# KAIST-AILab/SyncVSR

Measured on AMD Instinct MI355X. Metric: lip-clips/sec training (29x88x88), higher is better.
Workload: dtype bf16; 1 GPU; LRW training step (fwd+bwd+allreduce+clip+AdamW), ResNet18 + 6-layer 512-d encoder + vq audio-token CE head, random-init weights, N(0,1) clips 29x88x88, uniform tokens/labels; per_gpu_batch=32, global_batch=32, parallelism=dp1, hip_graph=False, enqueue=native step list

## Files before the change

### include/syncvsr_hip.h

```cpp
#ifndef SYNCVSR_HIP_H
#define SYNCVSR_HIP_H

#include <stdint.h>

#ifndef __HIP_PLATFORM_AMD__
typedef void* hipStream_t;
#else
#include <hip/hip_runtime_api.h>
#endif

#define SVSR_OK 0
#define SVSR_ERR_ARG 1001
#define SVSR_GRAD_ADD_DW 1
#define SVSR_GRAD_ADD_DB 2
#define SVSR_ERR_GROUP_OPEN 1003
#define SVSR_ERR_NO_GROUP 1004
#define SVSR_ERR_MASK_SIZE 1005

typedef struct svsr_wgrad_problem {
    const void* x; const void* dy; float* dw; float* dbias; const int* plan_dev; const int* meta;
    int Nimg; int in_pix; int Ci; int in_pitch; int Co; int out_pix; int out_pitch; int wt_taps;
} svsr_wgrad_problem;

typedef struct svsr_enc_layer {
// ... 40 lines not shown
int svsr_conv3x3_c64_stat_rows(int Nimg, int H, int W);
int64_t svsr_conv3x3_c64_pixtab(int Nimg, int H, int W, int* out, int64_t cap);
int svsr_conv3x3_c64(const void* in, const void* wt, void* out, const void* addend, float* stats, int Nimg, int H, int W, const int* dy, const int* dx, const int* tw, const int* pixtab, hipStream_t stream);

int svsr_igemm_dgrad_bn(const void* in, const void* wt, void* out, const void* addend, float* stats, const int* plan_dev, const int* meta, int Nimg, int in_pix, int Ci, int in_pitch, int Co, int out_pix, int out_pitch, int wt_taps, const void* y, const void* x, const float* mean, const float* rstd, const float* gamma, const float* beta, int act, hipStream_t stream);
int svsr_igemm_dgrad_relu(const void* in, const void* wt, void* out, float* stats, const int* plan_dev, const int* meta, int Nimg, int in_pix, int Ci, int in_pitch, int Co, int out_pix, int out_pitch, int wt_taps, const void* y, const float* zeros, const float* ones, float gscale, hipStream_t stream);
int svsr_conv3x3_c64_dgrad_bn(const void* in, const void* wt, void* out, const void* addend, float* stats, int Nimg, int H, int W, const int* dy, const int* dx, const int* tw, const void* y, const void* x, const float* mean, const float* rstd, const float* gamma, const float* beta, int act, const int* pixtab, hipStream_t stream);
int svsr_bn_bwd_from_stats(const void* g, const void* x, const float* mean, const float* rstd, const float* gamma, const float* stats, int nrows, float* coef, float* dgamma, float* dbeta, void* dx, int64_t npix, int C, hipStream_t stream);


int svsr_conv3x3_wgrad_plan(int Nimg, int H, int W, int Ci, int Co, int* splits, int64_t* part_floats);
int svsr_conv3x3_wgrad(const void* x, const void* dy, float* dw, int Nimg, int H, int W, int Ci, int Co, float* part, int64_t part_floats, hipStream_t stream);
int svsr_conv3x3_wgrad_v2(const void* x, const void* dy, float* dw, int Nimg, int H, int W, int Ci, int Co, float* part, int64_t part_floats, int mode, hipStream_t stream);

int svsr_stem_conv_fwd_stat_rows(int B, int T, int H, int W);
int64_t svsr_stem_conv_fwd_ws_bytes(int B, int T, int H, int W);
int svsr_stem_conv_fwd(const float* vid, const float* w, void* out, float* stats, int B, int T, int H, int W, void* ws, int64_t ws_bytes, hipStream_t stream);

int svsr_stem_conv_wgrad_plan(int B, int T, int H, int W, int* splits, int64_t* part_floats);
int svsr_stem_conv_wgrad(const float* vid, const void* dy, float* dw, int B, int T, int H, int W, int use_tr, float* part, int64_t part_floats, hipStream_t stream);

int svsr_stem_bwd_wgrad_ok(int B, int T, int H, int W);
int svsr_stem_bwd_wgrad(const float* vid, const void* gpool, const void* amax, const void* x, const float* mean, const float* rstd, const float* coef, float* dw, int B, int T, int H, int W, float* part, int64_t part_floats, hipStream_t stream);

int svsr_bn_finalize(const float* part, int nrows, int C, float count, float eps, float momentum, float* mean, float* rstd, float* running_mean, float* running_var, int64_t* num_batches_tracked, hipStream_t stream);

int svsr_bn_eval_prepare(const float* running_mean, const float* running_var, int C, float eps, float* mean, float* rstd, hipStream_t stream);

int svsr_bn_act_fwd(const void* x, const void* res, void* y, const float* mean, const float* rstd, const float* gamma, const float* beta, int64_t npix, int C, int act, hipStream_t stream);

int svsr_bn_act_bwd_rows(int64_t npix, int C);
int svsr_bn_act_bwd(const void* dy, const void* y, const void* x, const float* mean, const float* rstd, const float* gamma, float* slots, float* coef, float* dgamma, float* dbeta, void* dx, void* dres, int64_t npix, int C, int act, const float* beta, const void* res, hipStream_t stream);

int svsr_stem_bn_act_pool_fwd(const void* x, void* y, void* amax, const float* mean, const float* rstd, const float* gamma, const float* beta, int N, int Hc, int Wc, int Hp, int Wp, int C, int act, void* xwin, hipStream_t stream);

int svsr_stem_bn_act_pool_bwd_rows(int N, int Hc, int Wc, int C);
int svsr_stem_bn_act_pool_bwd(const void* dpool, const void* amax, const void* x, const float* mean, const float* rstd, const float* gamma, const float* beta, float* slots, float* coef, float* dgamma, float* dbeta, void* dx, int N, int Hc, int Wc, int Hp, int Wp, int C, int act, const void* xwin, void* gpool, hipStream_t stream);

int svsr_avgpool_fwd(const void* x, void* y, int64_t N, int HW, int C, hipStream_t stream);
int svsr_avgpool_bwd(const void* dy, void* dx, int64_t N, int HW, int C, hipStream_t stream);

int svsr_add_ln_fwd(const void* a, const void* r, const float* gamma, const float* beta, void* y, float* mean, float* rstd, int R, int D, float eps, hipStream_t stream);
int svsr_add_ln_bwd_rows(int R);
int svsr_add_ln_bwd(const void* dy, const void* a, const void* r, const float* gamma, const float* mean, const float* rstd, void* ds, float* dgamma, float* dbeta, int R, int D, const void* addend, float* part, hipStream_t stream);
int svsr_add_ln_bwd_partials(const void* dy, const void* a, const void* r, const float* gamma, const float* mean, const float* rstd, void* ds, int R, int D, const void* addend, float* part, hipStream_t stream);
int svsr_add_ln_bwd_branch(const void* dy, const void* a, const void* r, const float* gamma, const float* mean, const float* rstd, void* ds, int R, int D, const void* addend, float* part, void* ds2, float alpha2, const unsigned* drop_seed, unsigned drop_site, float drop_p, hipStream_t stream);
// ... 165 lines not shown
```

### syncvsr_amd/build.py

```python
from __future__ import annotations

import glob
import os
import subprocess
import sys
from concurrent.futures import ThreadPoolExecutor

PKG = os.path.dirname(os.path.abspath(__file__))
CSRC = os.path.join(PKG, "csrc")
LIB = os.path.join(PKG, "libsyncvsr_hip.so")
OBJ = os.path.join(PKG, "csrc", "_obj")
ARCH = "gfx950"
FLAGS = ["-O3", "-std=c++17", "-fPIC", f"--offload-arch={ARCH}", "-Wno-unused-value", "-ffp-contract=fast"]


def _hipcc() -> str:
    for c in ("hipcc", "/opt/rocm/bin/hipcc"):
        try:
            subprocess.run([c, "--version"], capture_output=True, check=True)
            return c
        except (OSError, subprocess.CalledProcessError):
            continue
    raise RuntimeError("hipcc not found (needed to build the gfx950 kernels)")


def sources() -> list[str]:
    return sorted(glob.glob(os.path.join(CSRC, "*.hip")))


def headers() -> list[str]:
    pub = os.path.join(os.path.dirname(os.path.dirname(os.path.abspath(__file__))), "include")
    return glob.glob(os.path.join(CSRC, "*.h")) + glob.glob(os.path.join(pub, "*.h"))


VARIANTS = {"": [], "syncdbg": ["-DSVSR_SYNC_DEBUG"], "p8stamp": ["-DSVSR_P8_STAMP"]}


def lib_path(variant: str = "") -> str:
    return os.path.join(PKG, f"libsyncvsr_hip_{variant}.so") if variant else LIB


def stale(variant: str = "") -> bool:
    lib = lib_path(variant)
    if not os.path.exists(lib):
        return True
    t = os.path.getmtime(lib)
    deps = sources() + headers()
    return any(os.path.getmtime(d) > t for d in deps)


def build(force: bool = False, verbose: bool = True, variant: str = "") -> str:
    LIB = lib_path(variant)
    OBJ = os.path.join(PKG, "csrc", "_obj" + ("_" + variant if variant else ""))
    if not force and not stale(variant):
        return LIB
    cc = _hipcc()
    os.makedirs(OBJ, exist_ok=True)
    srcs = sources()
# ... 28 lines not shown
```

### syncvsr_amd/csrc/stem.hip

```cpp
#include "common.h"

#define STEM_C 64
#define STEM_KROWS 36
#define STEM_WPITCH 296

typedef __attribute__((ext_vector_type(4))) unsigned v4u;
typedef __attribute__((ext_vector_type(2))) unsigned v2u;

struct StemFwdArgs {
    const float* vid;
    const float* w;
    bf16_t* out;
    float* stats;
    int B, T, H, W, Ho, Wo;
    int tiles_per_frame, total_tiles;
    int rows_in_max, WP;
};

__global__ __launch_bounds__(256) void k_stem_conv_fwd(const StemFwdArgs p) {
    extern __shared__ __attribute__((aligned(16))) unsigned char smem_raw[];
    bf16_t* sW = reinterpret_cast<bf16_t*>(smem_raw);
    bf16_t* sIn = sW + STEM_C * STEM_WPITCH;
    const int tid = threadIdx.x, lane = tid & 63, wave = tid >> 6;
    const int HoWo = p.Ho * p.Wo;
// ... 517 lines not shown
            }
        }
        if (nxt >= p.total_tiles) break;
    }
    float* dst = p.part + (long)blockIdx.x * (STEM_C * 245);
#pragma unroll
    for (int q = 0; q < 2; ++q) {
        const int k = (wave * 2 + q) * 32 + (lane & 31);
        if (k >= 245) continue;
#pragma unroll
        for (int i = 0; i < 2; ++i)
#pragma unroll
            for (int r = 0; r < 16; ++r) {
                const int c = i * 32 + (r & 3) + 8 * (r >> 2) + 4 * (lane >> 5);
                dst[c * 245 + k] = acc[i][q][r];
            }
    }
}


#define SBW_PR (SW_RB / 2 + 1)
#define SBW_NG 3

struct StemBwdWgradArgs {
    const float* vid;
    const bf16_t* x;
    const bf16_t* gpool;
    const unsigned char* amax;
    const float* mean;
    const float* rstd;
    const float* coef;
    float* part;
    int B, T, H, W, Ho, Wo, Hp, Wp;
    int WoP, PW, groups_per_frame, total_tiles;
};

template <int NDY, int NIN>
__global__ __launch_bounds__(256, 2) void k_stem_bwd_wgrad(const StemBwdWgradArgs p) {
    extern __shared__ __attribute__((aligned(16))) unsigned char smem_raw[];
    constexpr int nrows = 2 * SW_RB + 5;
    bf16_t* sDY = reinterpret_cast<bf16_t*>(smem_raw);
    bf16_t* sIn = sDY + SW_RB * p.WoP * SW_DPITCH;
    bf16_t* sG = sIn + 5 * nrows * 2 * p.PW;
    unsigned char* sM = reinterpret_cast<unsigned char*>(sG + SBW_PR * p.Wp * STEM_C);
    float* sC = reinterpret_cast<float*>(sM + SBW_PR * p.Wp * STEM_C);
    const int tid_k = threadIdx.x, lane = tid_k & 63, wave = tid_k >> 6;
    const int kg = lane >> 5;

    int kbase[2];
    bool kvalid[2];
#pragma unroll
    for (int q = 0; q < 2; ++q) {
        const int k = (wave * 2 + q) * 32 + (lane & 31);
        kvalid[q] = k < 245;
        const int kk = kvalid[q] ? k : 0;
        const int kt = kk / 49, kh = (kk % 49) / 7, kw = kk % 7;
        const int plane = (kw + 1) & 1, off = (kw + 1) >> 1;
        kbase[q] = ((kt * nrows + kh) * 2 + plane) * p.PW + off + kg * 8;
    }

    f32x16 acc[2][2];
#pragma unroll
    for (int i = 0; i < 2; ++i)
#pragma unroll
        for (int j = 0; j < 2; ++j)
#pragma unroll
            for (int r = 0; r < 16; ++r) acc[i][j][r] = 0.f;

    v4u xv[NDY], gv[SBW_NG];
    v2u mv[SBW_NG];
    f32x4 inv[NIN];
    const int dy_total = SW_RB * p.WoP * 8, g_total = SBW_PR * p.Wp * 8;
    const int nq = p.W >> 2, in_total = 5 * nrows * nq;
    const float inv_nq = 1.f / (float)nq;
    for (int d = tid_k; d < 5 * nrows * p.PW; d += 256) reinterpret_cast<unsigned*>(sIn)[d] = 0u;
    if (tid_k < STEM_C) {
        sC[0 * STEM_C + tid_k] = p.mean[tid_k]; sC[1 * STEM_C + tid_k] = p.rstd[tid_k];
        sC[2 * STEM_C + tid_k] = p.coef[tid_k]; sC[3 * STEM_C + tid_k] = p.coef[STEM_C + tid_k]; sC[4 * STEM_C + tid_k] = p.coef[2 * STEM_C + tid_k];
    }
    const float inv_wop = 1.f / (float)p.WoP;

    for (int tile = (int)blockIdx.x - (int)gridDim.x;; tile += gridDim.x) {
        const int nxt = tile + (int)gridDim.x;
        int rb = 0;
        int tid = tid_k;
        asm volatile("" : "+v"(tid));
        const int c0 = (tid & 7) * 8;
        if (tile >= 0) {
            const int gi = tile % p.groups_per_frame, y0 = gi * SW_RB, p_lo = y0 >> 1;
            rb = p.Ho - y0;
            if (rb > SW_RB) rb = SW_RB;
            __syncthreads();
#pragma unroll
            for (int i = 0; i < NDY; ++i) {
                const int e = tid + 256 * i;
                if (e < dy_total) *reinterpret_cast<v4u*>(sDY + (e >> 3) * SW_DPITCH + c0) = xv[i];
            }
#pragma unroll
            for (int i = 0; i < SBW_NG; ++i) {
                const int e = tid + 256 * i;
                if (e < g_total) {
                    *reinterpret_cast<v4u*>(sG + (e >> 3) * STEM_C + c0) = gv[i];
                    *reinterpret_cast<v2u*>(sM + (e >> 3) * STEM_C + c0) = mv[i];
                }
            }
#pragma unroll
            for (int i = 0; i < NIN; ++i) {
                const int it = tid + 256 * i, rr = (int)(((float)it + 0.5f) * inv_nq), l = it - rr * nq;
                if (it < in_total) {
                    bf16_t* dst = sIn + (long)rr * 2 * p.PW;
                    reinterpret_cast<unsigned*>(dst)[l + 1] = pack2bf(inv[i][0], inv[i][2]);
                    reinterpret_cast<unsigned*>(dst + p.PW)[l + 1] = pack2bf(inv[i][1], inv[i][3]);
                }
            }
            __syncthreads();
            float mu[8], rs[8], k0[8], k1[8], k2[8];
#pragma unroll
            for (int k = 0; k < 8; ++k) {
                mu[k] = sC[0 * STEM_C + c0 + k]; rs[k] = sC[1 * STEM_C + c0 + k];
                k0[k] = sC[2 * STEM_C + c0 + k]; k1[k] = sC[3 * STEM_C + c0 + k]; k2[k] = sC[4 * STEM_C + c0 + k];
            }
            const int nbw = (p.Wo + 1) >> 1;
#pragma unroll 1
            for (int e = tid; e < (SW_RB / 2) * nbw * 8; e += 256) {
                const int blk = e >> 3, rp = blk >= nbw ? 1 : 0, cp = blk - rp * nbw;
                if (2 * rp >= rb) continue;
                const bool row1 = 2 * rp + 1 < rb, col1 = 2 * cp + 1 < p.Wo;
                const bool ph1 = p_lo + rp + 1 < p.Hp, pw1 = cp + 1 < p.Wp;
                const int soA = (rp * p.Wp + cp) * STEM_C + c0, soB = soA + (pw1 ? STEM_C : 0);
                const int soC = soA + (ph1 ? p.Wp * STEM_C : 0), soD = soC + (pw1 ? STEM_C : 0);
                const uint2 mA = *reinterpret_cast<const uint2*>(sM + soA), mB = *reinterpret_cast<const uint2*>(sM + soB);
                const uint2 mC = *reinterpret_cast<const uint2*>(sM + soC), mD = *reinterpret_cast<const uint2*>(sM + soD);
                float gA[8], gB[8], gC[8], gD[8];
                unpack8(*reinterpret_cast<const u32x4*>(sG + soA), gA);
                unpack8(*reinterpret_cast<const u32x4*>(sG + soB), gB);
                unpack8(*reinterpret_cast<const u32x4*>(sG + soC), gC);
                unpack8(*reinterpret_cast<const u32x4*>(sG + soD), gD);
                const unsigned offB = pw1 ? 0u : 0xffu, offC = ph1 ? 0u : 0xffu, offD = (ph1 && pw1) ? 0u : 0xffu;
// ... 6 lines not shown
    {                                                                                                              \
        bf16_t* cell = sDY + ((2 * rp + dy_) * p.WoP + 2 * cp + dx_) * SW_DPITCH + c0;                            \
        float xf[8], a[8], ov[8];                                                                                  \
        unpack8(*reinterpret_cast<const u32x4*>(cell), xf);                                                        \
        _Pragma("unroll") for (int k = 0; k < 8; ++k) a[k] = 0.f;                                               \
        BODY                                                                                                       \
        _Pragma("unroll") for (int k = 0; k < 8; ++k) {                                                         \
            const float xh = (xf[k] - mu[k]) * rs[k];                                                              \
            ov[k] = k0[k] * (a[k] - k1[k] - xh * k2[k]);                                                           \
        }                                                                                                          \
        *reinterpret_cast<u32x4*>(cell) = pack8(ov);                                                               \
        __builtin_amdgcn_sched_barrier(0);                                                                         \
    }
                SBW_ELEM(0, 0, SBW_WIN(a, mA, gA, 4u))
                if (col1) SBW_ELEM(0, 1, SBW_WIN(a, mA, gA, 5u) SBW_WIN(a, mB, gB, 3u | offB))
                if (row1) {
                    SBW_ELEM(1, 0, SBW_WIN(a, mA, gA, 7u) SBW_WIN(a, mC, gC, 1u | offC))
                    if (col1) SBW_ELEM(1, 1, SBW_WIN(a, mA, gA, 8u) SBW_WIN(a, mB, gB, 6u | offB) SBW_WIN(a, mC, gC, 2u | offC) SBW_WIN(a, mD, gD, 0u | offD))
                }
#undef SBW_ELEM
#undef SBW_WIN
            }
            __syncthreads();
        }
        {
        if (nxt < p.total_tiles) {
            const int f = nxt / p.groups_per_frame, gi = nxt - f * p.groups_per_frame;
            const int b = f / p.T, t = f - b * p.T;
            const int y0 = gi * SW_RB, p_lo = y0 >> 1;
            int rbn = p.Ho - y0;
            if (rbn > SW_RB) rbn = SW_RB;
            const int row_base = 2 * y0 - 3;
#pragma unroll
            for (int i = 0; i < NDY; ++i) {
                const int e = tid + 256 * i, pos = e >> 3, yl = (int)(((float)pos + 0.5f) * inv_wop), w = pos - yl * p.WoP;
                const bool ok = e < dy_total && yl < rbn && w < p.Wo;
                xv[i] = *reinterpret_cast<const v4u*>(ok ? p.x + (((long)f * p.Ho + y0 + yl) * p.Wo + w) * STEM_C + c0
                                                           : reinterpret_cast<const bf16_t*>(g_stem_zero));
            }
            const int g_live = (p.Hp - p_lo) * p.Wp * 8;
#pragma unroll
            for (int i = 0; i < SBW_NG; ++i) {
                const int e = tid + 256 * i;
                const bool ok = e < g_total && e < g_live;
                const long o = (((long)f * p.Hp + p_lo) * p.Wp + (e >> 3)) * STEM_C + c0;
                gv[i] = *reinterpret_cast<const v4u*>(ok ? p.gpool + o : reinterpret_cast<const bf16_t*>(g_stem_zero));
                mv[i] = *reinterpret_cast<const v2u*>(ok ? p.amax + o : reinterpret_cast<const unsigned char*>(g_stem_zero));
            }
#pragma unroll
            for (int i = 0; i < NIN; ++i) {
                const int it = tid + 256 * i, rr = (int)(((float)it + 0.5f) * inv_nq), l = it - rr * nq;
                const int kt = rr / nrows, r = rr - kt * nrows;
                const int tt = t + kt - 2, iy = row_base + r;
                const bool ok = it < in_total && tt >= 0 && tt < p.T && iy >= 0 && iy < p.H;
                inv[i] = *reinterpret_cast<const f32x4*>(ok ? p.vid + (((long)b * p.T + tt) * p.H + iy) * p.W + 4 * l
                                                             : reinterpret_cast<const float*>(g_stem_zero));
            }
        }
        }
        if (tile < 0) {
            if (nxt >= p.total_tiles) break;
            continue;
        }

        for (int yl = 0; yl < rb; ++yl) {
            for (int xs = 0; xs < p.WoP; xs += 16) {
                const int pos0 = yl * p.WoP + xs;
                bf16x8 fa[2], fb[2];
                fa[0] = stem_frag_T<true>(sDY, 0, pos0, lane);
                fa[1] = stem_frag_T<true>(sDY, 32, pos0, lane);
#pragma unroll
                for (int q = 0; q < 2; ++q) {
                    const int a = kbase[q] + (2 * yl) * 2 * p.PW + xs;
                    const unsigned* src = reinterpret_cast<const unsigned*>(sIn + (a & ~1));
                    const unsigned sh = (a & 1) * 16;
                    const unsigned d0 = src[0], d1 = src[1], d2 = src[2], d3 = src[3], d4 = src[4];
                    u32x4 fr;
                    fr.x = kvalid[q] ? __builtin_amdgcn_alignbit(d1, d0, sh) : 0u;
                    fr.y = kvalid[q] ? __builtin_amdgcn_alignbit(d2, d1, sh) : 0u;
                    fr.z = kvalid[q] ? __builtin_amdgcn_alignbit(d3, d2, sh) : 0u;
                    fr.w = kvalid[q] ? __builtin_amdgcn_alignbit(d4, d3, sh) : 0u;
                    fb[q] = __builtin_bit_cast(bf16x8, fr);
                }
#pragma unroll
                for (int i = 0; i < 2; ++i)
#pragma unroll
                    for (int q = 0; q < 2; ++q)
                        acc[i][q] = __builtin_amdgcn_mfma_f32_32x32x16_bf16(fa[i], fb[q], acc[i][q], 0, 0, 0);
            }
        }
        if (nxt >= p.total_tiles) break;
    }
    float* dst = p.part + (long)blockIdx.x * (STEM_C * 245);
#pragma unroll
    for (int q = 0; q < 2; ++q) {
        const int k = (wave * 2 + q) * 32 + (lane & 31);
        if (k >= 245) continue;
#pragma unroll
        for (int i = 0; i < 2; ++i)
#pragma unroll
            for (int r = 0; r < 16; ++r) {
                const int c = i * 32 + (r & 3) + 8 * (r >> 2) + 4 * (lane >> 5);
                dst[c * 245 + k] = acc[i][q][r];
            }
    }
}

extern "C" {

static int stem_fwd_grid(int B, int T, int H, int W) {
    const long tiles = (long)(((H / 2) * (W / 2) + 127) / 128) * B * T;
    return (int)(tiles < 768 ? tiles : 768);
}
// ... 91 lines not shown
            lds_pipe = lds;
        }
        hipLaunchKernelGGL(k_stem_conv_wgrad_pipe<true>, dim3(grid), dim3(256), lds, stream, a);
    } else if (use_tr) hipLaunchKernelGGL(k_stem_conv_wgrad<true>, dim3(grid), dim3(256), lds, stream, a);
    else hipLaunchKernelGGL(k_stem_conv_wgrad<false>, dim3(grid), dim3(256), lds, stream, a);
    const int rc = svsr_check_launch();
    if (rc != SVSR_OK) return rc;
    return svsr_colsum_rows(part, grid, STEM_C * 245, dw, STEM_C * 245, nullptr, 0, 1, 1.0f, stream);
}


static bool stem_bwd_wgrad_shape(int B, int T, int H, int W, StemBwdWgradArgs& a, size_t& lds) {
    if ((H & 1) || (W & 3) || H < 8 || W < 8 || B < 1 || T < 1) return false;
    a.B = B; a.T = T; a.H = H; a.W = W; a.Ho = H / 2; a.Wo = W / 2;
    a.Hp = (a.Ho - 1) / 2 + 1; a.Wp = (a.Wo - 1) / 2 + 1;
    a.WoP = (a.Wo + 15) / 16 * 16;
    a.PW = a.WoP + 8;
    a.groups_per_frame = (a.Ho + SW_RB - 1) / SW_RB;
    a.total_tiles = a.groups_per_frame * B * T;
    lds = (size_t)SW_RB * a.WoP * SW_DPITCH * 2 + (size_t)5 * (2 * SW_RB + 5) * 2 * a.PW * 2 + (size_t)SBW_PR * a.Wp * STEM_C * 3 + 5 * STEM_C * sizeof(float);
    return a.PW / 2 <= 32 && SW_RB * a.WoP * 8 <= 8 * 256 && 5 * (2 * SW_RB + 5) * (W / 4) <= 8 * 256 && SBW_PR * a.Wp * 8 <= SBW_NG * 256 && lds <= 160 * 1024;
}

int svsr_stem_bwd_wgrad_ok(int B, int T, int H, int W) {
    StemBwdWgradArgs a;
    size_t lds;
    return stem_bwd_wgrad_shape(B, T, H, W, a, lds) ? 1 : 0;
}

int svsr_stem_bwd_wgrad(const float* vid, const void* gpool, const void* amax, const void* x, const float* mean, const float* rstd,
                        const float* coef, float* dw, int B, int T, int H, int W, float* part, int64_t part_floats, hipStream_t stream) {
    StemBwdWgradArgs a;
    size_t lds;
    if (!stem_bwd_wgrad_shape(B, T, H, W, a, lds)) return SVSR_ERR_ARG;
    const int grid = stem_wgrad_grid(B, T, H);
    if (part == nullptr || part_floats < (int64_t)grid * STEM_C * 245) return SVSR_ERR_ARG;
    a.vid = vid; a.x = (const bf16_t*)x; a.gpool = (const bf16_t*)gpool; a.amax = (const unsigned char*)amax;
    a.mean = mean; a.rstd = rstd; a.coef = coef; a.part = part;
    if (SW_RB * a.WoP * 8 > 6 * 256) return SVSR_ERR_ARG;
    const int v = (5 * (2 * SW_RB + 5) * (W / 4) <= 6 * 256) ? 0 : 1;
    const void* fn = v == 0 ? reinterpret_cast<const void*>(k_stem_bwd_wgrad<6, 6>) : reinterpret_cast<const void*>(k_stem_bwd_wgrad<6, 8>);
    static size_t lds_set[2] = {0, 0};
    if (lds > lds_set[v]) {
        (void)hipFuncSetAttribute(fn, hipFuncAttributeMaxDynamicSharedMemorySize, (int)lds);
        lds_set[v] = lds;
    }
    if (v == 0) hipLaunchKernelGGL((k_stem_bwd_wgrad<6, 6>), dim3(grid), dim3(256), lds, stream, a);
    else hipLaunchKernelGGL((k_stem_bwd_wgrad<6, 8>), dim3(grid), dim3(256), lds, stream, a);
    const int rc = svsr_check_launch();
    if (rc != SVSR_OK) return rc;
    return svsr_colsum_rows(part, grid, STEM_C * 245, dw, STEM_C * 245, nullptr, 0, 1, 1.0f, stream);
}

}
```

### syncvsr_amd/csrc/steplist.hip

```cpp
#include <stdlib.h>
#include <string.h>

#include <string>
#include <unordered_map>
#include <utility>
#include <vector>

#include "common.h"
#include "../../include/syncvsr_hip.h"

namespace {

typedef int64_t Slot;

template <typename T> struct FromSlot;
template <> struct FromSlot<int> { static int get(Slot s) { return (int)s; } };
template <> struct FromSlot<unsigned> { static unsigned get(Slot s) { return (unsigned)s; } };
template <> struct FromSlot<int64_t> { static int64_t get(Slot s) { return s; } };
template <> struct FromSlot<float> { static float get(Slot s) { double d; memcpy(&d, &s, sizeof d); return (float)d; } };
template <typename P> struct FromSlot<P*> { static P* get(Slot s) { return reinterpret_cast<P*>((uintptr_t)s); } };

template <typename... A, size_t... I>
int invoke(int (*fn)(A...), const Slot* s, std::index_sequence<I...>) { return fn(FromSlot<A>::get(s[I])...); }

template <typename... A>
int thunk_n(int (*)(A...)) { return (int)sizeof...(A); }

typedef int (*Thunk)(const Slot*);
struct Entry { Thunk call; int nargs; };

template <typename F, F fn> struct Bind;
template <typename... A, int (*fn)(A...)>
struct Bind<int (*)(A...), fn> {
    static int call(const Slot* s) { return invoke(fn, s, std::index_sequence_for<A...>{}); }
    static constexpr int nargs = (int)sizeof...(A);
};

#define SVSR_REG(f) {#f, Entry{&Bind<decltype(&f), &f>::call, Bind<decltype(&f), &f>::nargs}}

const std::unordered_map<std::string, Entry>& registry() {
    static const std::unordered_map<std::string, Entry> r = {
        SVSR_REG(svsr_colsum_rows), SVSR_REG(svsr_colsum_rows_multi), SVSR_REG(svsr_igemm_fwd), SVSR_REG(svsr_igemm_wgrad), SVSR_REG(svsr_conv3x3_c64),
        SVSR_REG(svsr_igemm_dgrad_bn), SVSR_REG(svsr_igemm_dgrad_relu), SVSR_REG(svsr_conv3x3_c64_dgrad_bn), SVSR_REG(svsr_bn_bwd_from_stats),
        SVSR_REG(svsr_conv3x3_wgrad), SVSR_REG(svsr_stem_conv_fwd), SVSR_REG(svsr_stem_conv_wgrad), SVSR_REG(svsr_stem_bwd_wgrad), SVSR_REG(svsr_bn_finalize),
        SVSR_REG(svsr_bn_eval_prepare), SVSR_REG(svsr_bn_act_fwd), SVSR_REG(svsr_bn_act_bwd), SVSR_REG(svsr_stem_bn_act_pool_fwd),
        SVSR_REG(svsr_stem_bn_act_pool_bwd), SVSR_REG(svsr_avgpool_fwd), SVSR_REG(svsr_avgpool_bwd), SVSR_REG(svsr_add_ln_fwd),
        SVSR_REG(svsr_add_ln_bwd), SVSR_REG(svsr_embed_ln_fwd), SVSR_REG(svsr_embed_bwd_scatter), SVSR_REG(svsr_rmsnorm_fwd),
        SVSR_REG(svsr_rmsnorm_bwd), SVSR_REG(svsr_rotary), SVSR_REG(svsr_geglu_fwd), SVSR_REG(svsr_geglu_bwd), SVSR_REG(svsr_xt_embed_fwd),
        SVSR_REG(svsr_xt_embed_bwd), SVSR_REG(svsr_bias_act_bwd), SVSR_REG(svsr_ce_fwd), SVSR_REG(svsr_ce_bwd), SVSR_REG(svsr_linear_ce_fwd), SVSR_REG(svsr_linear_ce_bwd), SVSR_REG(svsr_topk_acc),
        SVSR_REG(svsr_grad_sumsq), SVSR_REG(svsr_grad_sumsq_parts), SVSR_REG(svsr_adamw_step), SVSR_REG(svsr_adamw_range), SVSR_REG(svsr_cast_bf16), SVSR_REG(svsr_transpose_cast_multi),
        SVSR_REG(svsr_transpose_bf16_multi), SVSR_REG(svsr_fill_f32), SVSR_REG(svsr_clip_prep), SVSR_REG(svsr_mha_fwd), SVSR_REG(svsr_mha_bwd), SVSR_REG(svsr_mha_flash_fwd), SVSR_REG(svsr_mha_flash_bwd), SVSR_REG(svsr_mha_flash_bwd_parts), SVSR_REG(svsr_mha_pe_transpose),
        SVSR_REG(svsr_glu_dwconv_fwd), SVSR_REG(svsr_glu_dwconv_bwd), SVSR_REG(svsr_glu_dwconv_bwd_parts), SVSR_REG(svsr_ctc_fwd), SVSR_REG(svsr_ctc_grad),
        SVSR_REG(svsr_ctc_prefix_score), SVSR_REG(svsr_lrs_targets), SVSR_REG(svsr_embed_pos_fwd), SVSR_REG(svsr_embed_pos_bwd), SVSR_REG(svsr_ls_loss_fwd),
        SVSR_REG(svsr_ls_loss_bwd), SVSR_REG(svsr_scale_bf16), SVSR_REG(svsr_word_add), SVSR_REG(svsr_lincomb2), SVSR_REG(svsr_igemm_wgrad_group), SVSR_REG(svsr_enc_fwd), SVSR_REG(svsr_enc_bwd), SVSR_REG(svsr_lincomb3_ratio), SVSR_REG(svsr_add_ln_bwd_partials), SVSR_REG(svsr_add_ln_bwd_branch), SVSR_REG(svsr_bias_act_bwd_partials),
        SVSR_REG(svsr_memcpy_async), SVSR_REG(svsr_w2v_conv0), SVSR_REG(svsr_w2v_norm_gelu), SVSR_REG(svsr_w2v_quantize),
        SVSR_REG(svsr_igemm_wgrad_v2), SVSR_REG(svsr_igemm_wgrad_group_v2), SVSR_REG(svsr_conv3x3_wgrad_v2), SVSR_REG(svsr_fill_ranges),
        SVSR_REG(svsr_mha_table_fwd), SVSR_REG(svsr_lm_embed_fwd),
        SVSR_REG(svsr_beam_select), SVSR_REG(svsr_ctc_prefix_score_clips), SVSR_REG(svsr_mha_src_step_fwd), SVSR_REG(svsr_ctc_align),
        SVSR_REG(svsr_ctc_frame_best), SVSR_REG(svsr_ctc_collapse), SVSR_REG(svsr_edit_distance),
        SVSR_REG(svsr_tconv_fwd), SVSR_REG(svsr_tcn_se_fwd), SVSR_REG(svsr_tcn_norm_pool_fwd),
        SVSR_REG(svsr_tconv_fwd_save), SVSR_REG(svsr_tconv_epi_bwd), SVSR_REG(svsr_tconv_dgrad), SVSR_REG(svsr_tconv_wgrad), SVSR_REG(svsr_tcn_se_bwd),
        SVSR_REG(svsr_tcn_norm_pool_bwd), SVSR_REG(svsr_tcn_fold),
        SVSR_REG(svsr_lrs_clip_prep), SVSR_REG(svsr_wave_prep),
        SVSR_REG(svsr_lrw_clip_sums), SVSR_REG(svsr_lrw_clip_mix),
        SVSR_REG(svsr_vq_conv0_stats), SVSR_REG(svsr_vq_conv0_apply), SVSR_REG(svsr_vq_gn_partial), SVSR_REG(svsr_vq_gn_relu), SVSR_REG(svsr_vq_project),
        SVSR_REG(svsr_vq_assign),
    };
// ... 256 lines not shown
```

### syncvsr_amd/model.py

```python
from __future__ import annotations

import math
from typing import Any, Optional

import torch
import torch.nn as nn

from . import ops
from .config import Config, audio_codec_dims
from .init import buffer_specs, hidden_dim, init_state_dict, pad64, param_specs, phys_shape, resnet_block_specs, xt_dims

BF16 = torch.bfloat16


class _SideStream:

    def __init__(self) -> None:
        self.stream: Optional[torch.cuda.Stream] = None
        self.keep: list = []
        self._issuing = False
        self.enabled = False
        self.enabled_small = False

    def run(self, fn, *keep, small: bool = False) -> None:
# ... 614 lines not shown
    return ws["mean"], ws["rstd"]


def _conv_bn(st: _ParamStore, tape: dict, x: torch.Tensor, conv: str, bn: str, k: int, stride: int, pad: int, training: bool,
             res: Optional[torch.Tensor], act: int) -> torch.Tensor:
    o, n, shape = st.offsets[f"{conv}.weight"]
    w16 = st.w16[o : o + n].view(shape[0], k, k, shape[1])
    c, stats = ops.conv2d_fwd(x, w16, k, stride, pad, want_stats=training)
    mean, rstd = _bn_stats(st, bn, training, c.numel() // c.shape[-1], stats)
    y = ops.bn_act_fwd(c, res, mean, rstd, st.p32(f"{bn}.weight"), st.p32(f"{bn}.bias"), act)
    tape[conv] = dict(x=x, c=c, y=y, mean=mean, rstd=rstd, k=k, stride=stride, pad=pad, act=act, bn=bn, res=res)
    return y


def _trunk_blocks(model):
    for prefix, inp, planes, stride, down in resnet_block_specs():
        yield model.trunk_name + prefix[len("resnet"):], inp, planes, stride, down


def _frontend_forward(model, st: "_ParamStore", tape: dict, videos: torch.Tensor, training: bool) -> torch.Tensor:
    B, _, T, H, W = videos.shape
    N = B * T
    sc, sb, act = model.stem_name + ".0", model.stem_name + ".1", model.trunk_act
    c, stats = ops.stem_conv_fwd(videos, st.p32(f"{sc}.weight"), want_stats=training)
    mean, rstd = _bn_stats(st, sb, training, c.numel() // 64, stats)
    if training:
        x, amax, xwin = ops.stem_bn_gelu_pool_fwd(c, mean, rstd, st.p32(f"{sb}.weight"), st.p32(f"{sb}.bias"), model.stem_act, want_win=True)
    else:
        (x, amax), xwin = ops.stem_bn_gelu_pool_fwd(c, mean, rstd, st.p32(f"{sb}.weight"), st.p32(f"{sb}.bias"), model.stem_act), None
    tape["stem"] = dict(videos=videos, c=c, amax=amax, xwin=xwin, mean=mean, rstd=rstd, pooled_shape=tuple(x.shape))
    for prefix, inp, planes, stride, down in _trunk_blocks(model):
        xin = x
        if down and training and model._side.enabled:
            box: dict = {}
            model._side.run(lambda xin=xin, prefix=prefix, stride=stride: box.__setitem__(
                "idt", _conv_bn(st, tape, xin, f"{prefix}.downsample.0", f"{prefix}.downsample.1", 1, stride, 0, training, None, 0)), xin)
            o1 = _conv_bn(st, tape, xin, f"{prefix}.conv1", f"{prefix}.bn1", 3, stride, 1, training, None, act)
            model._side.join()
            idt = box["idt"]
        else:
            o1 = _conv_bn(st, tape, xin, f"{prefix}.conv1", f"{prefix}.bn1", 3, stride, 1, training, None, act)
            idt = _conv_bn(st, tape, xin, f"{prefix}.downsample.0", f"{prefix}.downsample.1", 1, stride, 0, training, None, 0) if down else xin
        x = _conv_bn(st, tape, o1, f"{prefix}.conv2", f"{prefix}.bn2", 3, 1, 1, training, idt, act)
    tape["trunk_out_shape"] = tuple(x.shape)
    return ops.avgpool_fwd(x)


def _frontend_backward(model, st: "_ParamStore", tape: dict, dfeats: torch.Tensor) -> None:
    act = model.trunk_act
    dx = ops.avgpool_bwd(dfeats, tape["trunk_out_shape"])
    fused = act in (1, 2) and ops.BN_BWD_FUSED
    dx_stats = None
    blocks = list(_trunk_blocks(model))
# ... 46 lines not shown
                dx, dx_stats = ops.conv2d_dgrad(dc1, w1t, 3, stride, 1, in_hw, addend=dxd), None
        elif tp is not None:
            dx, dx_stats = ops.conv2d_dgrad_bn(dc1, w1t, 3, stride, 1, in_hw, dres, tp_aux, tp["c"], tp["mean"], tp["rstd"], *tp_gb)
        else:
            dx, dx_stats = ops.conv2d_dgrad(dc1, w1t, 3, stride, 1, in_hw, addend=dres), None
        _ready(model, st, f"{prefix}.conv1.weight")
    ts = tape["stem"]
    if rec is not None:
        rec["stem"] = (dx.clone(), False)
    sc, sb = model.stem_name + ".0", model.stem_name + ".1"
    ws = st.bn[sb]
    fused = ts.get("xwin") is not None and ops.stem_bwd_wgrad_ok(ts["videos"])
    dconv = ops.stem_bn_gelu_pool_bwd(dx, ts["amax"], ts["c"], ts["mean"], ts["rstd"], st.p32(f"{sb}.weight"), st.p32(f"{sb}.bias"),
                                      ws["coef"], st.g32(f"{sb}.weight"), st.g32(f"{sb}.bias"), model.stem_act, xwin=ts.get("xwin"),
                                      want_dx=not fused)
    if fused:
        _flush_deferred(model)
        model._side.join()
        early = model._early_sumsq
        if early is not None and st.sumsq_head:
            with ops.window_group("tail"):
                model._side.run(lambda: ops.grad_sumsq_parts(st.grad, st.sumsq_head, st.numel - st.sumsq_head, early, 0, ops.SUMSQ_PARTS - 1))
            st.sumsq_tail_done = True
        ops.stem_bwd_wgrad(ts["videos"], dconv, ts["amax"], ts["c"], ts["mean"], ts["rstd"], ws["coef"], st.g32(f"{sc}.weight"))
    else:
        ops.stem_conv_wgrad(ts["videos"], dconv, st.g32(f"{sc}.weight"))
    _flush_deferred(model)
    model._side.join()
    _ready(model, st, None)


_ABLATE: frozenset = frozenset()


def _conv_wgrad(model, st: "_ParamStore", conv: str, t: dict, dc: torch.Tensor) -> None:
    if "conv_wgrad" in _ABLATE:
        return
    model._side.run(lambda: ops.conv2d_wgrad(t["x"], dc, st.g32(f"{conv}.weight"), t["k"], t["stride"], t["pad"]), dc)


def _lin_wgrad(model, x, dy, gw, gb, rows: int, K: int, N: int, x_pitch: int, dy_pitch: int) -> None:
    if "lin_wgrad" in _ABLATE:
        return
    group = model._wg_group
    if group is not None:
        group.append(dict(x=x, dy=dy, dw=gw, db=gb, rows=rows, K=K, N=N, x_pitch=x_pitch, dy_pitch=dy_pitch))
        return
# ... 452 lines not shown
```

### syncvsr_amd/ops.py

```python
from __future__ import annotations

import bisect
import ctypes
import os
import struct
from contextlib import contextmanager, nullcontext
from typing import Callable, Optional, Sequence

import torch

from . import _lib

BF16 = torch.bfloat16
BN_EPS = 1e-5
BN_MOMENTUM = 0.1
HALO_WGRAD = True


_DEV_INDEX: Optional[int] = None
STREAM_OVERRIDE: Optional[int] = None


def _stream() -> int:
    global _DEV_INDEX
# ... 858 lines not shown

        cv = _CONST_VECS[key] = tuple(torch.from_numpy(np.full(K, v, dtype=np.float32)).to(dy.device) for v in (0.0, 1.0))
    dz = torch.empty((rows, K), dtype=BF16, device=dy.device)
    plan = rows_plan(rows, 1, 0, 0, K)
    stats = torch.empty(plan.tiles * 2 * K, dtype=torch.float32, device=dy.device)
    _call("svsr_igemm_dgrad_relu", _p(dy), _p(w16t), _p(dz), _p(stats), plan.words.data_ptr(), plan.meta, rows, 1, Np, dy_pitch, K, 1, K, 1,
          _p(y), _p(cv[0]), _p(cv[1]), float(gscale), _stream(), label=plan.label + "+relu", flops=2.0 * rows * N * K)
    return dz, (stats, plan.tiles)


def linear_wgrad(x: torch.Tensor, dy: torch.Tensor, dw: torch.Tensor, *, rows: int, K: int, N: int, x_pitch: int, dy_pitch: int,
                 seq: Optional[tuple[int, int, int]] = None, db: Optional[torch.Tensor] = None, mode: Optional[int] = None) -> None:
    if seq is None:
        plan, geo = wgrad_rows_plan(rows, 1, 0, 0, K, N, db is not None), dict(Nimg=rows, in_pix=1, out_pix=1)
    else:
        S, s0, n = seq
        plan, geo = wgrad_rows_plan(rows // n, n, s0, 0, K, N, db is not None), dict(Nimg=rows // n, in_pix=S, out_pix=n)
    igemm_wgrad(plan, x, dy, dw, Ci=K, in_pitch=x_pitch, Co=N, out_pitch=dy_pitch, db=db, flops=2.0 * rows * N * K, mode=mode, **geo)


_STEM_WS: dict = {}


def stem_conv_fwd(videos: torch.Tensor, w: torch.Tensor, want_stats: bool = False, use_ws: bool = True, out: Optional[torch.Tensor] = None):
    B, C, T, H, W = videos.shape
    assert C == 1 and videos.dtype == torch.float32 and videos.is_contiguous()
    if out is None:
        out = torch.empty((B * T, H // 2, W // 2, 64), dtype=BF16, device=videos.device)
    assert out.shape == (B * T, H // 2, W // 2, 64) and out.dtype == BF16 and out.is_contiguous()
    stats = st = None
    if want_stats:
        rows = _query("svsr_stem_conv_fwd_stat_rows", B, T, H, W)[0]
        stats = scratch(rows * 2 * 64)
        st = (stats, rows)
    nws = _query("svsr_stem_conv_fwd_ws_bytes", B, T, H, W)[0] if use_ws else 0
    ws = None
    if nws:
        key = (videos.device, _stream())
        ws = _STEM_WS.get(key)
        if ws is None or ws.numel() < nws:
            if ws is not None:
                _SCRATCH_KEEP.append(ws)
            ws = _STEM_WS[key] = torch.empty(nws, dtype=torch.uint8, device=videos.device)
    _call("svsr_stem_conv_fwd", _p(videos), _p(w), _p(out), _p(stats), B, T, H, W, _p(ws), nws, _stream(),
          label="k_stem_conv_fwd", flops=2.0 * B * T * (H // 2) * (W // 2) * 64 * 245)
    return out, st


def stem_conv_wgrad(videos: torch.Tensor, dy: torch.Tensor, dw: torch.Tensor, use_tr: bool = True) -> None:
    B, _, T, H, W = videos.shape
    _, nfl = _query("svsr_stem_conv_wgrad_plan", B, T, H, W)
    _call("svsr_stem_conv_wgrad", _p(videos), _p(dy), _p(dw), B, T, H, W, int(use_tr), _p(scratch(nfl)), nfl, _stream(),
          label=f"k_stem_conv_wgrad<{'true' if use_tr else 'false'}>", flops=2.0 * B * T * (H // 2) * (W // 2) * 64 * 245)


ACT_NONE, ACT_RELU, ACT_GELU, ACT_SWISH = 0, 1, 1, 2


def stem_bn_gelu_pool_fwd(x: torch.Tensor, mean, rstd, gamma, beta, act: int = ACT_GELU, want_win: bool = False, out: Optional[torch.Tensor] = None):
    N, Hc, Wc, C = x.shape
    Hp, Wp = (Hc - 1) // 2 + 1, (Wc - 1) // 2 + 1
    y = torch.empty((N, Hp, Wp, C), dtype=BF16, device=x.device) if out is None else out
    assert y.shape == (N, Hp, Wp, C) and y.dtype == BF16 and y.is_contiguous()
    amax = torch.empty((N, Hp, Wp, C), dtype=torch.uint8, device=x.device)
    xwin = torch.empty((N, Hp, Wp, C), dtype=BF16, device=x.device) if want_win else None
    _call("svsr_stem_bn_act_pool_fwd", _p(x), _p(y), _p(amax), _p(mean), _p(rstd), _p(gamma), _p(beta), N, Hc, Wc, Hp, Wp, C, act, _p(xwin), _stream())
    return (y, amax, xwin) if want_win else (y, amax)


def stem_bn_gelu_pool_bwd(dpool, amax, x, mean, rstd, gamma, beta, coef, dgamma, dbeta, act: int = ACT_GELU, xwin=None, want_dx: bool = True,
                          out: Optional[torch.Tensor] = None):
    N, Hc, Wc, C = x.shape
    _, Hp, Wp, _ = dpool.shape
    assert want_dx or xwin is not None
    dx = (torch.empty_like(x) if out is None else out) if want_dx else None
    assert dx is None or (dx.shape == x.shape and dx.dtype == x.dtype and dx.is_contiguous())
    slots = scratch(_query("svsr_stem_bn_act_pool_bwd_rows", N, Hc, Wc, C)[0] * 2 * C)
    gpool = torch.empty_like(dpool) if xwin is not None else None
    _call("svsr_stem_bn_act_pool_bwd", _p(dpool), _p(amax), _p(x), _p(mean), _p(rstd), _p(gamma), _p(beta), _p(slots), _p(coef),
          _p(dgamma), _p(dbeta), _p(dx), N, Hc, Wc, Hp, Wp, C, act, _p(xwin), _p(gpool), _stream())
    return dx if want_dx else gpool


def stem_bwd_wgrad_ok(videos: torch.Tensor) -> bool:
    B, _, T, H, W = videos.shape
    return bool(_lib.load().svsr_stem_bwd_wgrad_ok(B, T, H, W))


def stem_bwd_wgrad(videos: torch.Tensor, gpool, amax, x, mean, rstd, coef, dw: torch.Tensor) -> None:
    B, _, T, H, W = videos.shape
    _, nfl = _query("svsr_stem_conv_wgrad_plan", B, T, H, W)
    _call("svsr_stem_bwd_wgrad", _p(videos), _p(gpool), _p(amax), _p(x), _p(mean), _p(rstd), _p(coef), _p(dw), B, T, H, W, _p(scratch(nfl)), nfl,
          _stream(), label="k_stem_bwd_wgrad", flops=2.0 * B * T * (H // 2) * (W // 2) * 64 * 245)


def bn_finalize(stats, C: int, count: int, mean, rstd, running_mean=None, running_var=None, nbt=None) -> None:
    part, rows = stats
    _call("svsr_bn_finalize", _p(part), rows, C, float(count), BN_EPS, BN_MOMENTUM, _p(mean), _p(rstd), _p(running_mean), _p(running_var),
          _p(nbt), _stream())


def bn_eval_prepare(running_mean, running_var, mean, rstd) -> None:
    _call("svsr_bn_eval_prepare", _p(running_mean), _p(running_var), running_mean.numel(), BN_EPS, _p(mean), _p(rstd), _stream())


def bn_act_fwd(x, res, mean, rstd, gamma, beta, act: int) -> torch.Tensor:
    C = x.shape[-1]
    y = torch.empty_like(x)
    _call("svsr_bn_act_fwd", _p(x), _p(res), _p(y), _p(mean), _p(rstd), _p(gamma), _p(beta), x.numel() // C, C, act, _stream())
    return y


def bn_act_bwd(dy, y, x, mean, rstd, gamma, coef, dgamma, dbeta, act: int, want_dres: bool, beta=None, res=None):
    C = x.shape[-1]
    dx = torch.empty_like(x)
    dres = torch.empty_like(x) if want_dres else None
# ... 1102 lines not shown
```

Measured before the change: 6918 clips/s.

## Reuse forward stem bf16 row workspace in stem backward weight-gradient

The forward stem conv workspace, which holds padded bf16 rows of the input video, is now kept alive per step instead of living in a shared cached buffer. The backward stem wgrad kernel reads these bf16 rows in place of the fp32 video. That halves the input bytes it loads and lets it split even and odd columns with byte permutes instead of converting fp32 to bf16. It costs an extra workspace allocation each training step and relies on the workspace layout matching the W+8 padded rows. Optional timestamp instrumentation is also added, compiled only in a separate build variant.

```diff
diff --git a/include/syncvsr_hip.h b/include/syncvsr_hip.h
--- a/include/syncvsr_hip.h
+++ b/include/syncvsr_hip.h
@@ -86,6 +86,7 @@
 
 int svsr_stem_bwd_wgrad_ok(int B, int T, int H, int W);
 int svsr_stem_bwd_wgrad(const float* vid, const void* gpool, const void* amax, const void* x, const float* mean, const float* rstd, const float* coef, float* dw, int B, int T, int H, int W, float* part, int64_t part_floats, hipStream_t stream);
+int svsr_stem_bwd_wgrad_v2(const float* vid, const void* vid16, const void* gpool, const void* amax, const void* x, const float* mean, const float* rstd, const float* coef, float* dw, int B, int T, int H, int W, float* part, int64_t part_floats, hipStream_t stream);
 
 int svsr_bn_finalize(const float* part, int nrows, int C, float count, float eps, float momentum, float* mean, float* rstd, float* running_mean, float* running_var, int64_t* num_batches_tracked, hipStream_t stream);
 
diff --git a/syncvsr_amd/build.py b/syncvsr_amd/build.py
--- a/syncvsr_amd/build.py
+++ b/syncvsr_amd/build.py
@@ -33,7 +33,8 @@
     return glob.glob(os.path.join(CSRC, "*.h")) + glob.glob(os.path.join(pub, "*.h"))
 
 
-VARIANTS = {"": [], "syncdbg": ["-DSVSR_SYNC_DEBUG"], "p8stamp": ["-DSVSR_P8_STAMP"]}
+VARIANTS = {"": [], "syncdbg": ["-DSVSR_SYNC_DEBUG"], "p8stamp": ["-DSVSR_P8_STAMP"],
+            "stemstamp": ["-DSVSR_STEM_STAMP"]}
 
 
 def lib_path(variant: str = "") -> str:
diff --git a/syncvsr_amd/csrc/stem.hip b/syncvsr_amd/csrc/stem.hip
--- a/syncvsr_amd/csrc/stem.hip
+++ b/syncvsr_amd/csrc/stem.hip
@@ -563,8 +563,21 @@
 #define SBW_PR (SW_RB / 2 + 1)
 #define SBW_NG 3
 
+#ifdef SVSR_STEM_STAMP
+__device__ unsigned long long g_stem_stamp[2][8];
+#define SBW_STAMP(slot)                                                                                                   \
+    {                                                                                                                     \
+        const long long t_now = __builtin_amdgcn_s_memtime();                                                             \
+        if (stamp_row >= 0 && tid_k == 0) atomicAdd(&g_stem_stamp[stamp_row][slot], (unsigned long long)(t_now - t_stamp)); \
+        t_stamp = t_now;                                                                                                  \
+    }
+#else
+#define SBW_STAMP(slot)
+#endif
+
 struct StemBwdWgradArgs {
     const float* vid;
+    const bf16_t* vid16;
     const bf16_t* x;
     const bf16_t* gpool;
     const unsigned char* amax;
@@ -576,6 +589,7 @@
     int WoP, PW, groups_per_frame, total_tiles;
 };
 
+#define SBW_NIN16 4
 template <int NDY, int NIN>
 __global__ __launch_bounds__(256, 2) void k_stem_bwd_wgrad(const StemBwdWgradArgs p) {
     extern __shared__ __attribute__((aligned(16))) unsigned char smem_raw[];
@@ -596,7 +610,7 @@
         kvalid[q] = k < 245;
         const int kk = kvalid[q] ? k : 0;
         const int kt = kk / 49, kh = (kk % 49) / 7, kw = kk % 7;
-        const int plane = (kw + 1) & 1, off = (kw + 1) >> 1;
+        const int plane = (kw + 1) & 1, off = ((kw + 1) >> 1) - ((p.vid16 != nullptr && plane == 0) ? 1 : 0);
         kbase[q] = ((kt * nrows + kh) * 2 + plane) * p.PW + off + kg * 8;
     }
 
@@ -608,6 +622,10 @@
 #pragma unroll
             for (int r = 0; r < 16; ++r) acc[i][j][r] = 0.f;
 
+    static_assert(NIN >= SBW_NIN16, "the bf16 pieces live in the fp32 pieces' registers");
+    const bool rows16 = p.vid16 != nullptr;
+    const int cpr = (p.W + 8) >> 3, in16_total = 5 * nrows * cpr;
+    const float inv_cpr = 1.f / (float)cpr;
     v4u xv[NDY], gv[SBW_NG];
     v2u mv[SBW_NG];
     f32x4 inv[NIN];
@@ -620,6 +638,10 @@
         sC[2 * STEM_C + tid_k] = p.coef[tid_k]; sC[3 * STEM_C + tid_k] = p.coef[STEM_C + tid_k]; sC[4 * STEM_C + tid_k] = p.coef[2 * STEM_C + tid_k];
     }
     const float inv_wop = 1.f / (float)p.WoP;
+#ifdef SVSR_STEM_STAMP
+    const int stamp_row = blockIdx.x == 0 ? 0 : (blockIdx.x == gridDim.x / 2 ? 1 : -1);
+    long long t_stamp = __builtin_amdgcn_s_memtime();
+#endif
 
     for (int tile = (int)blockIdx.x - (int)gridDim.x;; tile += gridDim.x) {
         const int nxt = tile + (int)gridDim.x;
@@ -631,7 +653,12 @@
             const int gi = tile % p.groups_per_frame, y0 = gi * SW_RB, p_lo = y0 >> 1;
             rb = p.Ho - y0;
             if (rb > SW_RB) rb = SW_RB;
+            SBW_STAMP(7)
             __syncthreads();
+#ifdef SVSR_STEM_STAMP
+            asm volatile("s_waitcnt vmcnt(0)" ::: "memory");
+#endif
+            SBW_STAMP(0)
 #pragma unroll
             for (int i = 0; i < NDY; ++i) {
                 const int e = tid + 256 * i;
@@ -645,6 +672,21 @@
                     *reinterpret_cast<v2u*>(sM + (e >> 3) * STEM_C + c0) = mv[i];
                 }
             }
+            if (rows16) {
+#pragma unroll
+                for (int i = 0; i < SBW_NIN16; ++i) {
+                    const int it = tid + 256 * i, rr = (int)(((float)it + 0.5f) * inv_cpr), j = it - rr * cpr;
+                    if (it < in16_total) {
+                        const v4u d = __builtin_bit_cast(v4u, inv[i]);
+                        bf16_t* dst = sIn + (long)rr * 2 * p.PW;
+                        v2u ev, od;
+                        ev[0] = __builtin_amdgcn_perm(d[1], d[0], 0x07060302u); ev[1] = __builtin_amdgcn_perm(d[3], d[2], 0x07060302u);
+                        od[0] = __builtin_amdgcn_perm(d[1], d[0], 0x05040100u); od[1] = __builtin_amdgcn_perm(d[3], d[2], 0x05040100u);
+                        reinterpret_cast<v2u*>(dst)[j] = ev;
+                        reinterpret_cast<v2u*>(dst + p.PW)[j] = od;
+                    }
+                }
+            } else {
 #pragma unroll
             for (int i = 0; i < NIN; ++i) {
                 const int it = tid + 256 * i, rr = (int)(((float)it + 0.5f) * inv_nq), l = it - rr * nq;
@@ -654,7 +696,9 @@
                     reinterpret_cast<unsigned*>(dst + p.PW)[l + 1] = pack2bf(inv[i][1], inv[i][3]);
                 }
             }
+            }
             __syncthreads();
+            SBW_STAMP(1)
             float mu[8], rs[8], k0[8], k1[8], k2[8];
 #pragma unroll
             for (int k = 0; k < 8; ++k) {
@@ -707,6 +751,7 @@
 #undef SBW_WIN
             }
             __syncthreads();
+            SBW_STAMP(2)
         }
         {
         if (nxt < p.total_tiles) {
@@ -732,6 +777,17 @@
                 gv[i] = *reinterpret_cast<const v4u*>(ok ? p.gpool + o : reinterpret_cast<const bf16_t*>(g_stem_zero));
                 mv[i] = *reinterpret_cast<const v2u*>(ok ? p.amax + o : reinterpret_cast<const unsigned char*>(g_stem_zero));
             }
+            if (rows16) {
+#pragma unroll
+                for (int i = 0; i < SBW_NIN16; ++i) {
+                    const int it = tid + 256 * i, rr = (int)(((float)it + 0.5f) * inv_cpr), j = it - rr * cpr;
+                    const int kt = rr / nrows, r = rr - kt * nrows;
+                    const int tt = t + kt - 2, iy = row_base + r;
+                    const bool ok = it < in16_total && tt >= 0 && tt < p.T && iy >= 0 && iy < p.H;
+                    inv[i] = *reinterpret_cast<const f32x4*>(ok ? reinterpret_cast<const float*>(p.vid16 + (((long)b * p.T + tt) * p.H + iy) * (p.W + 8) + 8 * j)
+                                                                 : reinterpret_cast<const float*>(g_stem_zero));
+                }
+            } else {
 #pragma unroll
             for (int i = 0; i < NIN; ++i) {
                 const int it = tid + 256 * i, rr = (int)(((float)it + 0.5f) * inv_nq), l = it - rr * nq;
@@ -741,12 +797,14 @@
                 inv[i] = *reinterpret_cast<const f32x4*>(ok ? p.vid + (((long)b * p.T + tt) * p.H + iy) * p.W + 4 * l
                                                              : reinterpret_cast<const float*>(g_stem_zero));
             }
+            }
         }
         }
         if (tile < 0) {
             if (nxt >= p.total_tiles) break;
             continue;
         }
+        SBW_STAMP(3)
 
         for (int yl = 0; yl < rb; ++yl) {
             for (int xs = 0; xs < p.WoP; xs += 16) {
@@ -774,6 +832,11 @@
                         acc[i][q] = __builtin_amdgcn_mfma_f32_32x32x16_bf16(fa[i], fb[q], acc[i][q], 0, 0, 0);
             }
         }
+#ifdef SVSR_STEM_STAMP
+        asm volatile("s_nop 0" ::"v"(acc[0][0][0]), "v"(acc[1][1][15]));
+        SBW_STAMP(4)
+        if (stamp_row >= 0 && tid_k == 0) atomicAdd(&g_stem_stamp[stamp_row][5], 1ull);
+#endif
         if (nxt >= p.total_tiles) break;
     }
     float* dst = p.part + (long)blockIdx.x * (STEM_C * 245);
@@ -911,6 +974,10 @@
     return a.PW / 2 <= 32 && SW_RB * a.WoP * 8 <= 8 * 256 && 5 * (2 * SW_RB + 5) * (W / 4) <= 8 * 256 && SBW_PR * a.Wp * 8 <= SBW_NG * 256 && lds <= 160 * 1024;
 }
 
+int svsr_stem_bwd_wgrad_v2(const float* vid, const void* vid16, const void* gpool, const void* amax, const void* x, const float* mean,
+                           const float* rstd, const float* coef, float* dw, int B, int T, int H, int W, float* part, int64_t part_floats,
+                           hipStream_t stream);
+
 int svsr_stem_bwd_wgrad_ok(int B, int T, int H, int W) {
     StemBwdWgradArgs a;
     size_t lds;
@@ -919,9 +986,17 @@
 
 int svsr_stem_bwd_wgrad(const float* vid, const void* gpool, const void* amax, const void* x, const float* mean, const float* rstd,
                         const float* coef, float* dw, int B, int T, int H, int W, float* part, int64_t part_floats, hipStream_t stream) {
+    return svsr_stem_bwd_wgrad_v2(vid, nullptr, gpool, amax, x, mean, rstd, coef, dw, B, T, H, W, part, part_floats, stream);
+}
+
+int svsr_stem_bwd_wgrad_v2(const float* vid, const void* vid16, const void* gpool, const void* amax, const void* x, const float* mean,
+                           const float* rstd, const float* coef, float* dw, int B, int T, int H, int W, float* part, int64_t part_floats,
+                           hipStream_t stream) {
     StemBwdWgradArgs a;
     size_t lds;
     if (!stem_bwd_wgrad_shape(B, T, H, W, a, lds)) return SVSR_ERR_ARG;
+    if (vid16 != nullptr && ((W & 7) || ((uintptr_t)vid16 & 15) || 5 * (2 * SW_RB + 5) * ((W + 8) / 8) > SBW_NIN16 * 256)) return SVSR_ERR_ARG;
+    a.vid16 = (const bf16_t*)vid16;
     const int grid = stem_wgrad_grid(B, T, H);
     if (part == nullptr || part_floats < (int64_t)grid * STEM_C * 245) return SVSR_ERR_ARG;
     a.vid = vid; a.x = (const bf16_t*)x; a.gpool = (const bf16_t*)gpool; a.amax = (const unsigned char*)amax;
@@ -941,4 +1016,12 @@
     return svsr_colsum_rows(part, grid, STEM_C * 245, dw, STEM_C * 245, nullptr, 0, 1, 1.0f, stream);
 }
 
-}
+#ifdef SVSR_STEM_STAMP
+int svsr_debug_stem_stamps(long long* out16) {
+    if (hipMemcpyFromSymbol(out16, HIP_SYMBOL(g_stem_stamp), 16 * sizeof(long long)) != hipSuccess) return SVSR_ERR_LAUNCH;
+    const long long z[16] = {0};
+    return (int)hipMemcpyToSymbol(HIP_SYMBOL(g_stem_stamp), z, sizeof z);
+}
+#endif
+
+}
diff --git a/syncvsr_amd/csrc/steplist.hip b/syncvsr_amd/csrc/steplist.hip
--- a/syncvsr_amd/csrc/steplist.hip
+++ b/syncvsr_amd/csrc/steplist.hip
@@ -42,7 +42,7 @@
     static const std::unordered_map<std::string, Entry> r = {
         SVSR_REG(svsr_colsum_rows), SVSR_REG(svsr_colsum_rows_multi), SVSR_REG(svsr_igemm_fwd), SVSR_REG(svsr_igemm_wgrad), SVSR_REG(svsr_conv3x3_c64),
         SVSR_REG(svsr_igemm_dgrad_bn), SVSR_REG(svsr_igemm_dgrad_relu), SVSR_REG(svsr_conv3x3_c64_dgrad_bn), SVSR_REG(svsr_bn_bwd_from_stats),
-        SVSR_REG(svsr_conv3x3_wgrad), SVSR_REG(svsr_stem_conv_fwd), SVSR_REG(svsr_stem_conv_wgrad), SVSR_REG(svsr_stem_bwd_wgrad), SVSR_REG(svsr_bn_finalize),
+        SVSR_REG(svsr_conv3x3_wgrad), SVSR_REG(svsr_stem_conv_fwd), SVSR_REG(svsr_stem_conv_wgrad), SVSR_REG(svsr_stem_bwd_wgrad), SVSR_REG(svsr_stem_bwd_wgrad_v2), SVSR_REG(svsr_bn_finalize),
         SVSR_REG(svsr_bn_eval_prepare), SVSR_REG(svsr_bn_act_fwd), SVSR_REG(svsr_bn_act_bwd), SVSR_REG(svsr_stem_bn_act_pool_fwd),
         SVSR_REG(svsr_stem_bn_act_pool_bwd), SVSR_REG(svsr_avgpool_fwd), SVSR_REG(svsr_avgpool_bwd), SVSR_REG(svsr_add_ln_fwd),
         SVSR_REG(svsr_add_ln_bwd), SVSR_REG(svsr_embed_ln_fwd), SVSR_REG(svsr_embed_bwd_scatter), SVSR_REG(svsr_rmsnorm_fwd),
diff --git a/syncvsr_amd/model.py b/syncvsr_amd/model.py
--- a/syncvsr_amd/model.py
+++ b/syncvsr_amd/model.py
@@ -660,13 +660,17 @@
     B, _, T, H, W = videos.shape
     N = B * T
     sc, sb, act = model.stem_name + ".0", model.stem_name + ".1", model.trunk_act
-    c, stats = ops.stem_conv_fwd(videos, st.p32(f"{sc}.weight"), want_stats=training)
+    rows16 = None
+    if training and ops.stem_bwd_wgrad_ok(videos):
+        c, stats, rows16 = ops.stem_conv_fwd(videos, st.p32(f"{sc}.weight"), want_stats=True, keep_rows=True)
+    else:
+        c, stats = ops.stem_conv_fwd(videos, st.p32(f"{sc}.weight"), want_stats=training)
     mean, rstd = _bn_stats(st, sb, training, c.numel() // 64, stats)
     if training:
         x, amax, xwin = ops.stem_bn_gelu_pool_fwd(c, mean, rstd, st.p32(f"{sb}.weight"), st.p32(f"{sb}.bias"), model.stem_act, want_win=True)
     else:
         (x, amax), xwin = ops.stem_bn_gelu_pool_fwd(c, mean, rstd, st.p32(f"{sb}.weight"), st.p32(f"{sb}.bias"), model.stem_act), None
-    tape["stem"] = dict(videos=videos, c=c, amax=amax, xwin=xwin, mean=mean, rstd=rstd, pooled_shape=tuple(x.shape))
+    tape["stem"] = dict(videos=videos, rows16=rows16, c=c, amax=amax, xwin=xwin, mean=mean, rstd=rstd, pooled_shape=tuple(x.shape))
     for prefix, inp, planes, stride, down in _trunk_blocks(model):
         xin = x
         if down and training and model._side.enabled:
@@ -759,7 +763,8 @@
             with ops.window_group("tail"):
                 model._side.run(lambda: ops.grad_sumsq_parts(st.grad, st.sumsq_head, st.numel - st.sumsq_head, early, 0, ops.SUMSQ_PARTS - 1))
             st.sumsq_tail_done = True
-        ops.stem_bwd_wgrad(ts["videos"], dconv, ts["amax"], ts["c"], ts["mean"], ts["rstd"], ws["coef"], st.g32(f"{sc}.weight"))
+        ops.stem_bwd_wgrad(ts["videos"], dconv, ts["amax"], ts["c"], ts["mean"], ts["rstd"], ws["coef"], st.g32(f"{sc}.weight"),
+                           rows16=ts.get("rows16"))
     else:
         ops.stem_conv_wgrad(ts["videos"], dconv, st.g32(f"{sc}.weight"))
     _flush_deferred(model)
diff --git a/syncvsr_amd/ops.py b/syncvsr_amd/ops.py
--- a/syncvsr_amd/ops.py
+++ b/syncvsr_amd/ops.py
@@ -904,7 +904,8 @@
 _STEM_WS: dict = {}
 
 
-def stem_conv_fwd(videos: torch.Tensor, w: torch.Tensor, want_stats: bool = False, use_ws: bool = True, out: Optional[torch.Tensor] = None):
+def stem_conv_fwd(videos: torch.Tensor, w: torch.Tensor, want_stats: bool = False, use_ws: bool = True, out: Optional[torch.Tensor] = None,
+                  keep_rows: bool = False):
     B, C, T, H, W = videos.shape
     assert C == 1 and videos.dtype == torch.float32 and videos.is_contiguous()
     if out is None:
@@ -917,7 +918,9 @@
         st = (stats, rows)
     nws = _query("svsr_stem_conv_fwd_ws_bytes", B, T, H, W)[0] if use_ws else 0
     ws = None
-    if nws:
+    if nws and keep_rows:
+        ws = torch.empty(nws, dtype=torch.uint8, device=videos.device)
+    elif nws:
         key = (videos.device, _stream())
         ws = _STEM_WS.get(key)
         if ws is None or ws.numel() < nws:
@@ -926,6 +929,8 @@
             ws = _STEM_WS[key] = torch.empty(nws, dtype=torch.uint8, device=videos.device)
     _call("svsr_stem_conv_fwd", _p(videos), _p(w), _p(out), _p(stats), B, T, H, W, _p(ws), nws, _stream(),
           label="k_stem_conv_fwd", flops=2.0 * B * T * (H // 2) * (W // 2) * 64 * 245)
+    if keep_rows:
+        return out, st, ws
     return out, st
 
 
@@ -969,11 +974,13 @@
     return bool(_lib.load().svsr_stem_bwd_wgrad_ok(B, T, H, W))
 
 
-def stem_bwd_wgrad(videos: torch.Tensor, gpool, amax, x, mean, rstd, coef, dw: torch.Tensor) -> None:
+def stem_bwd_wgrad(videos: torch.Tensor, gpool, amax, x, mean, rstd, coef, dw: torch.Tensor, rows16: Optional[torch.Tensor] = None) -> None:
     B, _, T, H, W = videos.shape
     _, nfl = _query("svsr_stem_conv_wgrad_plan", B, T, H, W)
-    _call("svsr_stem_bwd_wgrad", _p(videos), _p(gpool), _p(amax), _p(x), _p(mean), _p(rstd), _p(coef), _p(dw), B, T, H, W, _p(scratch(nfl)), nfl,
-          _stream(), label="k_stem_bwd_wgrad", flops=2.0 * B * T * (H // 2) * (W // 2) * 64 * 245)
+    if rows16 is not None:
+        assert rows16.is_contiguous() and rows16.numel() * rows16.element_size() >= B * T * H * (W + 8) * 2
+    _call("svsr_stem_bwd_wgrad_v2", _p(videos), _p(rows16), _p(gpool), _p(amax), _p(x), _p(mean), _p(rstd), _p(coef), _p(dw), B, T, H, W,
+          _p(scratch(nfl)), nfl, _stream(), label="k_stem_bwd_wgrad", flops=2.0 * B * T * (H // 2) * (W // 2) * 64 * 245)
 
 
 def bn_finalize(stats, C: int, count: int, mean, rstd, running_mean=None, running_var=None, nbt=None) -> None:
```

Result: no change. 6951 clips/s (median of 5 runs) (+0.5%).
